# UM-Applied-Algorithms-Lab/AWRY

Measured on NVIDIA B200. Metric: count queries/s, higher is better.
Workload: dtype u32

## Files before the change

### awry_b200/csrc/batch.cu

```cuda
#include "host.hpp"

using namespace awry;
using namespace awry::host;

namespace awry {
namespace host {


static bool trace_on() {
  static const bool on = getenv("AWRY_B200_TRACE") != nullptr;
  return on;
}
static void trace_mark(const char* what, long long i = -1) {
  if (!trace_on()) return;
  static const auto t_origin = std::chrono::steady_clock::now();
  fprintf(stderr, "[trace] %10.3f ms  %s %lld\n",
          std::chrono::duration<double, std::milli>(std::chrono::steady_clock::now() - t_origin).count(), what, i);
}
struct GpuTrace {
  struct Ev {
    cudaEvent_t e;
    const char* what;
    long long i;
  };
// ... 160 lines not shown
  host_parallel_blocks(size_t(nb), [&](size_t b) {
    if (!ok.load(std::memory_order_relaxed)) return;
    const uint64_t lo = b * BLK, hi = std::min(nq, lo + BLK);
    uint64_t bad = 0;
    for (uint64_t i = lo; i <= hi; i++) bad |= off[i] ^ (first + i * l);
    if (bad) ok.store(false, std::memory_order_relaxed);
  });
  return ok.load();
}

void enqueue_search(const awry_index* ix, Replica& r, PackBalance& bal, Workspace* ws, const QuerySource& qs,
                    const Chunk& c, SearchOut mode, bool may_pack = true, bool probe_link = false, bool copy_flag = true,
                    void* d_out_override = nullptr) {
  const uint64_t nq = c.q1 - c.q0, nbytes = c.b1 - c.b0;
  const size_t out_elem = mode == OUT_COUNT_U64 ? 8 : mode == OUT_RANGE_U64 ? 16 : sp_cnt_bytes(r.view);
  const int ush = packed_unit_shift(ix->alphabet);
  Workspace::grow_dev(ws->d_qbytes, ws->d_qbytes_cap, size_t(nbytes) + 16);
  Workspace::grow_dev(ws->d_qoff, ws->d_qoff_cap, size_t(nq) + 1);
  Workspace::grow_dev(ws->d_qwords, ws->d_qwords_cap, size_t(packed_words(ix->alphabet, nq, nbytes)));
  Workspace::grow_dev(ws->d_out, ws->d_out_cap, size_t(nq) * out_elem);
  Workspace::grow_dev(ws->d_defer, ws->d_defer_cap, defer_words(nq));
  const uint64_t* src_o = qs.qoff + c.q0;
  uint64_t* const d_words = ws->d_qwords - 4 * (c.b0 >> ush);
  ws->link_probe_bytes = 0;
  uint64_t uni_len = 0;
  const bool uniform = offsets_are_uniform(src_o, nq, uni_len);
  auto upload_offsets = [&] {
    if (uniform) {
      CU(launch_fill_offsets(ws->d_qoff, c.b0, uni_len, nq, ws->st));
    } else {
      CU(cudaMemcpyAsync(ws->d_qoff, src_o, (nq + 1) * 8, cudaMemcpyHostToDevice, ws->st));
      g_prof.h2d += (nq + 1) * 8;
    }
  };
  auto stage_offsets = [&] {
    if (qs.pinned || uniform) return;
    Workspace::grow_host(ws->h_qoff, ws->h_qoff_cap, size_t(nq) + 1);
    parallel_memcpy(ws->h_qoff, src_o, (nq + 1) * 8);
    src_o = ws->h_qoff;
  };
  if (qs.crumbs) {
    const uint64_t cb0 = c.b0 >> 2, cb1 = (c.b1 + 3) >> 2;
    const size_t pbytes = size_t(cb1 - cb0);
    const uint8_t* src_c = qs.crumbs + cb0;
    const uint64_t* e_lo = std::lower_bound(qs.exc, qs.exc + qs.n_exc, c.b0 << 8);
    const uint64_t* e_hi = std::lower_bound(e_lo, qs.exc + qs.n_exc, c.b1 << 8);
// ... 59 lines not shown
    } else {
      if (!qs.pinned) {
        Workspace::grow_host(ws->h_qbytes, ws->h_qbytes_cap, size_t(nbytes) + 16);
        parallel_memcpy(ws->h_qbytes, src_b, nbytes);
        src_b = ws->h_qbytes;
      }
      stage_offsets();
      const bool probe = probe_link && qs.pinned && nbytes >= (8u << 20);
      if (probe) {
        if (!ws->ev_a) {
          CU(cudaEventCreate(&ws->ev_a));
          CU(cudaEventCreate(&ws->ev_b));
        }
        CU(cudaEventRecord(ws->ev_a, ws->st));
      }
      if (nbytes) CU(cudaMemcpyAsync(ws->d_qbytes, src_b, nbytes, cudaMemcpyHostToDevice, ws->st));
      if (probe) {
        CU(cudaEventRecord(ws->ev_b, ws->st));
        ws->link_probe_bytes = nbytes;
      }
      upload_offsets();
      g_prof.h2d += nbytes;
      CU(cudaMemsetAsync(ws->d_flag, 0xff, 8, ws->st));
      {
        ProfScope p(2, r.device, ws->st);
        CU(launch_pack(ix->alphabet, ws->d_qbytes - c.b0, ws->d_qoff, nq, d_words, c.b0, c.b1, ws->d_flag, ws->st));
      }
    }
  }
  gpu_mark(ws->st, "packed on device", (long long)c.q0);
  {
    ProfScope p(0, r.device, ws->st);
    SearchVariant v = current_variant();
    v.avg_len = uint32_t(std::min<uint64_t>(nbytes / std::max<uint64_t>(1, nq), 1u << 30));
    v.b_lo = c.b0;
    v.b_hi = c.b1;
    v.locate_positions = mode == OUT_SP_CNT_U32 && locate_positions_ok(r.view, v);
    ws->sp_cnt_positions = v.locate_positions;
    ws->gpu_probe_bytes = 0;
    const bool time_kernel = qs.pinned && !qs.crumbs && nbytes >= (8u << 20);
    if (time_kernel) {
      if (!ws->ev_s0) {
        CU(cudaEventCreate(&ws->ev_s0));
        CU(cudaEventCreate(&ws->ev_s1));
      }
      CU(cudaEventRecord(ws->ev_s0, ws->st));
    }
    CU(launch_search(r.view, d_words, ws->d_qoff, nq, mode, d_out_override ? d_out_override : ws->d_out, ws->d_defer, v,
                     r.sm_count, ws->st));
    if (time_kernel) {
      CU(cudaEventRecord(ws->ev_s1, ws->st));
      ws->gpu_probe_bytes = nbytes;
    }
  }
  gpu_mark(ws->st, "searched", (long long)c.q0);
  if (copy_flag) CU(cudaMemcpyAsync(ws->h_flag, ws->d_flag, 8, cudaMemcpyDeviceToHost, ws->st));
  trace_mark("  search enqueued, queries", (long long)nq);
}

[[noreturn]] void fail_bad_query(unsigned long long code, uint64_t q_base) {
  const unsigned long long q = q_base + (code >> 1);
  if ((code & 1) == BAD_OFFSETS)
    fail(AWRY_ERR_INVALID_ARG, "query offsets are not monotone at query %llu (its bytes lie outside the batch)", q);
  fail(AWRY_ERR_INVALID_QUERY,
       "query %llu is empty or contains a sentinel ('$'/'#'): the reference panics on it "
       "(fm_index.rs:406, bwt.rs:127)", q);
}

void check_flag(Workspace* ws, const Chunk& c) {
  if (*ws->h_flag != ~0ull) fail_bad_query(*ws->h_flag, c.q0);
}

// ... 969 lines not shown
  });
}

int awry_count_device(const awry_index* ix, int replica, const uint8_t* d_qbytes, const uint64_t* d_qoff, uint64_t nq,
                      uint64_t* d_counts, void* cuda_stream) {
  return guarded([&] {
    need(ix);
    if (replica < 0 || size_t(replica) >= ix->reps.size()) fail(AWRY_ERR_INVALID_ARG, "replica out of range");
    if (nq == 0) return;
    if (!d_qbytes || !d_qoff || !d_counts) fail(AWRY_ERR_INVALID_ARG, "null argument");
    Replica& r = *ix->reps[size_t(replica)];
    DeviceGuard dg(r.device);
    cudaStream_t st = static_cast<cudaStream_t>(cuda_stream);
    uint64_t ends[2] = {0, 0};
    CU(cudaMemcpyAsync(&ends[0], d_qoff, 8, cudaMemcpyDeviceToHost, st));
    CU(cudaMemcpyAsync(&ends[1], d_qoff + nq, 8, cudaMemcpyDeviceToHost, st));
    CU(cudaStreamSynchronize(st));
    if (ends[1] < ends[0]) fail(AWRY_ERR_INVALID_ARG, "query offsets are not monotone");
    const int sh = packed_unit_shift(ix->alphabet);
    uint64_t words = 4 * (nq + ((ends[1] >> sh) - (ends[0] >> sh)) + 2) + 32;
    uint64_t* d_qwords = nullptr;
    CU(cudaMallocAsync(reinterpret_cast<void**>(&d_qwords), words * 8 + defer_words(nq) * 4, st));
    uint32_t* d_defer = reinterpret_cast<uint32_t*>(d_qwords + words);
    {
      ProfScope p(2, r.device, st);
      CU(launch_pack(ix->alphabet, d_qbytes, d_qoff, nq, d_qwords - 4 * (ends[0] >> sh), ends[0], ends[1], r.d_async_flag, st));
    }
    {
      ProfScope p(0, r.device, st);
      SearchVariant v = current_variant();
      v.avg_len = uint32_t(std::min<uint64_t>((ends[1] - ends[0]) / nq, 1u << 30));
      v.b_lo = ends[0];
      v.b_hi = ends[1];
      CU(launch_search(r.view, d_qwords - 4 * (ends[0] >> sh), d_qoff, nq, OUT_COUNT_U64, d_counts, d_defer, v, r.sm_count, st));
    }
    CU(cudaFreeAsync(d_qwords, st));
  });
}

int awry_locate_device(const awry_index* ix, int replica, const uint8_t* d_qbytes, const uint64_t* d_qoff, uint64_t nq,
                       uint32_t flags, uint64_t* d_hit_off, awry_hit** d_hits, uint64_t* n_hits, void* cuda_stream) {
  return guarded([&] {
    need(ix);
    if (replica < 0 || size_t(replica) >= ix->reps.size()) fail(AWRY_ERR_INVALID_ARG, "replica out of range");
    if (!d_hit_off || !d_hits || !n_hits) fail(AWRY_ERR_INVALID_ARG, "null argument");
    *d_hits = nullptr;
    *n_hits = 0;
    if (nq == 0) return;
    if (!d_qbytes || !d_qoff) fail(AWRY_ERR_INVALID_ARG, "null argument");
    Replica& r = *ix->reps[size_t(replica)];
    DeviceGuard dg(r.device);
    cudaStream_t st = static_cast<cudaStream_t>(cuda_stream);
    uint64_t ends[2] = {0, 0};
    CU(cudaMemcpyAsync(&ends[0], d_qoff, 8, cudaMemcpyDeviceToHost, st));
    CU(cudaMemcpyAsync(&ends[1], d_qoff + nq, 8, cudaMemcpyDeviceToHost, st));
    CU(cudaStreamSynchronize(st));
    if (ends[1] < ends[0]) fail(AWRY_ERR_INVALID_ARG, "query offsets are not monotone");
    const int sh = packed_unit_shift(ix->alphabet);
    Workspace* ws = r.acquire();
    try {
      uint64_t words = 4 * (nq + ((ends[1] >> sh) - (ends[0] >> sh)) + 2) + 32;
      Workspace::grow_dev(ws->d_qwords, ws->d_qwords_cap, size_t(words));
      Workspace::grow_dev(ws->d_out, ws->d_out_cap, size_t(nq) * sp_cnt_bytes(r.view));
      Workspace::grow_dev(ws->d_defer, ws->d_defer_cap, defer_words(nq));
      {
        ProfScope p(2, r.device, st);
        CU(launch_pack(ix->alphabet, d_qbytes, d_qoff, nq, ws->d_qwords - 4 * (ends[0] >> sh), ends[0], ends[1], r.d_async_flag, st));
      }
      {
        ProfScope p(0, r.device, st);
        SearchVariant v = current_variant();
        v.avg_len = uint32_t(std::min<uint64_t>((ends[1] - ends[0]) / nq, 1u << 30));
        v.b_lo = ends[0];
        v.b_hi = ends[1];
        v.locate_positions = locate_positions_ok(r.view, v);
        ws->sp_cnt_positions = v.locate_positions;
        CU(launch_search(r.view, ws->d_qwords - 4 * (ends[0] >> sh), d_qoff, nq, OUT_SP_CNT_U32, ws->d_out, ws->d_defer, v, r.sm_count, st));
      }
      uint64_t n = 0;
      uint64_t* h = locate_chunk_device(ix, r, ws, nq, flags, d_hit_off, &n, st);
      CU(cudaStreamSynchronize(st));
      *d_hits = reinterpret_cast<awry_hit*>(h);
      *n_hits = n;
    } catch (...) {
      cudaStreamSynchronize(st);
      r.release(ws);
      throw;
    }
    r.release(ws);
  });
}

int awry_count_batch_hamming(const awry_index* ix, const uint8_t* qbytes, const uint64_t* qoff, uint64_t nq,
                             uint32_t max_mismatches, uint64_t* counts) {
  return guarded([&] {
    need(ix);
    if (max_mismatches > AWRY_HAMMING_MAX) fail(AWRY_ERR_INVALID_ARG, "max_mismatches must be 0 .. %d", AWRY_HAMMING_MAX);
    if (nq == 0) return;
    if (!qbytes || !qoff || !counts) fail(AWRY_ERR_INVALID_ARG, "null argument");
    hamming_check_index(ix);
// ... 150 lines not shown
```

### awry_b200/csrc/kernels.cu

```cuda
#include <atomic>
#include <cstdio>
#include <cub/device/device_scan.cuh>
#include <cub/device/device_segmented_sort.cuh>
#include <thrust/iterator/counting_iterator.h>
#include <thrust/iterator/transform_iterator.h>

#include "kernels_common.cuh"

namespace awry {

std::atomic<uint64_t> g_launches{0};
uint64_t kernel_launch_count() { return g_launches.load(); }
void kernel_launch_count_reset() { g_launches.store(0); }


__constant__ uint8_t c_ascii_to_dsym[2][256];
__constant__ uint8_t c_amino_code_to_idx[32];

static uint8_t host_ascii_to_ref_index(int alphabet, uint8_t ch) {
  if (ch >= 'a' && ch <= 'z') ch = uint8_t(ch - 'a' + 'A');
  if (ch == '$' || ch == '#') return 0;
  if (alphabet == 0) {
    switch (ch) {
      case 'A': return 1;
// ... 480 lines not shown
  return cleanup(e);
}


template <int ALPHA>
__device__ __forceinline__ uint64_t pack_word_bytes(const uint8_t* __restrict__ src, uint32_t len, uint32_t first,
                                                    const uint8_t* lut, bool& bad) {
  constexpr int BITS = ALPHA == 0 ? 4 : 8;
  constexpr int SPW = 64 / BITS;
  constexpr uint32_t SENT = ALPHA == 0 ? DNA_SENTINEL : AMINO_SENTINEL;
  uint64_t word = 0;
#pragma unroll 4
  for (int t = 0; t < SPW; t++) {
    uint32_t si = first + t;
    if (si < len) {
      uint32_t d = lut[src[len - 1 - si]];
      bad |= d == SENT;
      word |= uint64_t(d) << (BITS * t);
    }
  }
  return word;
}

template <int ALPHA, int PL = 8>
__global__ void __launch_bounds__(256)
    pack_kernel(const uint8_t* __restrict__ qbytes, const uint64_t* __restrict__ qoff, uint64_t nq,
                uint64_t* __restrict__ qwords, uint64_t b_lo, uint64_t b_hi, unsigned long long* first_bad) {
  constexpr int SPW = ALPHA == 0 ? 16 : 8;
  constexpr int LOG_SPW = ALPHA == 0 ? 4 : 3;
  constexpr int UNIT_SHIFT = ALPHA == 0 ? 6 : 5;
  __shared__ uint8_t lut[256];
  lut[threadIdx.x] = c_ascii_to_dsym[ALPHA][threadIdx.x];
  __syncthreads();
  constexpr int LOG_PL = PL == 8 ? 3 : PL == 4 ? 2 : 1;
  const uint32_t sub = threadIdx.x & (PL - 1);
  const uint64_t ngroups = (gridDim.x * uint64_t(blockDim.x)) >> LOG_PL;
  for (uint64_t q = (blockIdx.x * uint64_t(blockDim.x) + threadIdx.x) >> LOG_PL; q < nq; q += ngroups) {
    const uint64_t o0 = qoff[q], o1 = qoff[q + 1];
    if (o0 < b_lo || o1 > b_hi || o1 < o0 || o1 - o0 >= (1ull << 32)) {
      if (sub == 0) atomicMin(first_bad, bad_query_code(q, BAD_OFFSETS));
      continue;
    }
    if (o1 == o0) {
      if (sub == 0) atomicMin(first_bad, bad_query_code(q, BAD_QUERY));
      continue;
    }
// ... 1 lines not shown
    const uint32_t nwords = (len + SPW - 1) >> LOG_SPW;
    uint64_t* const dst = qwords + 4 * (q + (o0 >> UNIT_SHIFT));
    const uint8_t* const src = qbytes + o0;
    bool bad = false;
#pragma unroll 4
    for (uint32_t wi = sub; wi < nwords; wi += PL) {
      const uint32_t first = wi << LOG_SPW;
      uint64_t word;
      bool done = false;
      if (ALPHA == 0 && len >= 16) {
        const uint32_t have = len - first;
        const uint32_t drop = have >= 16 ? 0 : 16 - have;
        const uint8_t* p = src + (have >= 16 ? have - 16 : 0);
        const uint32_t sh = uint32_t(reinterpret_cast<uintptr_t>(p) & 3);
        const uint32_t* a = reinterpret_cast<const uint32_t*>(p - sh);
        uint32_t u[5];
#pragma unroll
        for (int j = 0; j < 4; j++) u[j] = __ldg(a + j);
        u[4] = sh ? __ldg(a + 4) : 0u;
        uint32_t nibs[4];
        bool clean = true;
#pragma unroll
        for (int j = 0; j < 4; j++) {
          uint32_t w4 = __funnelshift_r(u[j], u[j + 1], 8 * sh);
          uint32_t rev = __byte_perm(w4, 0, 0x0123);
          uint32_t up = rev & 0xDFDFDFDFu;
          uint32_t x4 = (up >> 1) & 0x03030303u;
          uint32_t c4 = x4 ^ ((x4 >> 1) & 0x01010101u);
          uint32_t sel = c4 | (c4 >> 4);
          uint32_t nib = (sel & 0xffu) | ((sel >> 8) & 0xff00u);
          clean &= up == __byte_perm(0x54474341u, 0, nib);
          nibs[j] = nib;
        }
        if (clean) {
          word = (uint64_t(nibs[1] | (nibs[0] << 16)) << 32) | uint64_t(nibs[3] | (nibs[2] << 16));
          word >>= 4 * drop;
          done = true;
        }
      }
      if (!done) word = pack_word_bytes<ALPHA>(src, len, first, lut, bad);
      dst[wi] = word;
    }
    if (bad) atomicMin(first_bad, bad_query_code(q, BAD_QUERY));
  }
}

cudaError_t launch_pack(int alphabet, const uint8_t* d_qbytes, const uint64_t* d_qoff, uint64_t nq,
                        uint64_t* d_qwords, uint64_t b_lo, uint64_t b_hi, unsigned long long* d_first_bad,
                        cudaStream_t s) {
  if (nq == 0) return cudaSuccess;
  const uint64_t avg_len = b_hi != ~0ull && b_hi > b_lo ? (b_hi - b_lo) / nq : 150;
  const int pl = alphabet != 0 ? 8 : avg_len >= 48 ? 4 : 2;
  uint64_t threads = nq * uint64_t(pl);
  unsigned grid = unsigned(std::min<uint64_t>((threads + 255) / 256, 148 * 64));
  if (alphabet == 0 && pl == 4)
// ... 553 lines not shown
          for (uint32_t sec = s_first + sub; sec <= s_last; sec += 4) {
            AWRY_CHK(uint64_t(sec) * 32 + 31 < ix.n_rtext);
            const u32x8 t = ldg256(ix.rtext + size_t(sec) * 32);
            bad |= in_ring ? text_sector_mismatch<true>(t, ring, sec, rb0, done, len)
                           : text_sector_mismatch<false>(t, qwords + ubase, sec, rb0, done, len);
          }
          ok = !__any_sync(gmask, bad != 0u);
        }
        if (sub == 0) {
          if (MODE == OUT_COUNT_U64)
            reinterpret_cast<uint64_t*>(out)[cur] = ok ? 1ull : 0ull;
          else
            reinterpret_cast<uint2*>(out)[cur] = ok ? make_uint2(p - left, CNT_AT_TEXT_POS) : make_uint2(1u, 0u);
        }
        cur = NONE;
        left = 0;
      }
    }
  }
}

constexpr int WAVE_MAX_STEPS = 6;

template <int MODE, int TPB, int MINB>
__global__ void __launch_bounds__(TPB, MINB)
    search_dna_wave_kernel(IndexView ix, const uint64_t* __restrict__ qwords, const uint64_t* __restrict__ qoff,
                           uint64_t nq, void* __restrict__ out, uint32_t* __restrict__ defer, uint32_t ticket_sz,
                           ByteRange br) {
  constexpr uint32_t FULL = 0xffffffffu;
  enum : uint32_t { W_NONE = 0, W_RUN = 1, W_EMPTY = 2 };
  __shared__ uint64_t s_q[TPB / 4][16];
  const uint32_t lane = threadIdx.x & 31, sub = lane & 3, gbase = lane - sub, gmask = 0xfu << gbase, grp = lane >> 2;
  uint64_t* const ring = s_q[threadIdx.x >> 2];
  const uint32_t nq32 = uint32_t(nq);
  uint32_t* const ticket = defer + nq + 1;
  uint32_t* const rest = defer + nq + 2;
  uint32_t pn = 0, pe = 0;
  uint32_t ahead = 0;
  if (lane == 0) ahead = atomicAdd(ticket, ticket_sz);
  for (;;) {
    if (pn == pe) {
      uint32_t t = ahead;
      if (lane == 0 && t < nq32) ahead = atomicAdd(ticket, ticket_sz);
      t = __shfl_sync(FULL, t, 0);
      if (t >= nq32) break;
      pn = t;
      pe = t + (nq32 - t < ticket_sz ? nq32 - t : ticket_sz);
    }
    const uint32_t q = pn + grp;
    uint32_t st = q < pe ? W_RUN : W_NONE;
    pn = pe - pn > 8u ? pn + 8u : pe;

    uint64_t ov = 0;
    if (st == W_RUN) ov = __ldg(qoff + q + (sub & 1));
    const uint64_t o0 = __shfl_sync(FULL, ov, gbase), o1 = __shfl_sync(FULL, ov, gbase + 1);
    const uint32_t len = st == W_RUN ? checked_len(o0, o1, br) : 0u;
    if (st == W_RUN && len == 0) st = W_EMPTY;
    const uint32_t nwords = (len + 15) >> 4;
    if (st == W_RUN && nwords > 16) {
      if (sub == 0) rest[2 + atomicAdd(rest, 1u)] = q;
      st = W_NONE;
    }
    uint32_t amb = 0;
    __syncwarp();
    if (st == W_RUN && 4 * sub < nwords) {
      const uint32_t ubase = 4 * (q + uint32_t(o0 >> 6));
      AWRY_CHK_QWORDS(ubase + 4 * sub, br, nq, 6);
      const u32x8 t = ldg256(qwords + ubase + 4 * sub);
#pragma unroll
      for (int j = 0; j < 4; j++) {
        ring[4 * sub + j] = uint64_t(t.v[2 * j]) | (uint64_t(t.v[2 * j + 1]) << 32);
        if (4 * sub + j < nwords) amb |= (t.v[2 * j] | t.v[2 * j + 1]) & 0xCCCCCCCCu;
      }
    }
    const uint32_t amb_groups = __ballot_sync(FULL, amb != 0);
    __syncwarp();
    if (st == W_RUN && (amb_groups & gmask) != 0) {
      if (sub == 0) defer[1 + atomicAdd(defer, 1u)] = q;
      st = W_NONE;
    }
    uint32_t sp = 1, ep = 0, left = 0;
    if (st == W_RUN) {
      const uint32_t k = ix.kmer_len;
      const uint64_t w = ring[0];
      if (k != 0 && len >= k) {
        const uint64_t idx = kmer_index(w, k);
        AWRY_CHK(idx < ix.n_table);
        const uint2 r = __ldg(ix.table + idx);
        sp = r.x;
        ep = r.y;
        left = len - k;
      } else {
        const uint32_t c = uint32_t(w) & 15u;
        sp = ix.c_lo[c];
        ep = ix.c_hi[c];
        left = len - 1;
      }
    }
#pragma unroll 1
    for (int it = 0; it <= WAVE_MAX_STEPS; it++) {
      const bool active = st == W_RUN && left != 0 && sp <= ep && !(sp == ep && left >= VERIFY_MIN_LEFT);
      if (!__any_sync(FULL, active)) break;
      if (it == WAVE_MAX_STEPS) {
        if (active) {
          if (sub == 0) rest[2 + atomicAdd(rest, 1u)] = q;
          st = W_NONE;
        }
        break;
      }
      const uint32_t pos = len - left;
      const uint8_t* const rb8 = reinterpret_cast<const uint8_t*>(ring);
      const uint32_t qb = rb8[(pos >> 1) & 127];
      const bool two = left >= 2;
      const uint32_t pa = sp - 1, pb = ep;
      uint32_t ra = 0, rb = 0, base = 0;
      if (active) {
        if (two) {
          const uint32_t q2 = ((qb | (uint32_t(rb8[((pos >> 1) + 1) & 127]) << 8)) >> (4 * (pos & 1))) & 0xffu;
          const uint32_t pair = ((q2 & 3u) << 2) | (q2 >> 4);
          const uint32_t ba = __umulhi(pa, 0xAAAAAAABu) >> 6, bb = __umulhi(pb, 0xAAAAAAABu) >> 6;
          AWRY_CHK(uint64_t(ba) * PAIR_BLOCK_UINT4 + 7 < ix.n_pair_u4 && uint64_t(bb) * PAIR_BLOCK_UINT4 + 7 < ix.n_pair_u4);
          const u32x8 x = ldg256(ix.pair_blocks + size_t(ba) * PAIR_BLOCK_UINT4 + 2 * sub);
          u32x8 y = x;
          if (bb != ba) y = ldg256(ix.pair_blocks + size_t(bb) * PAIR_BLOCK_UINT4 + 2 * sub);
          PairSlice s = pair_slice(x, sub, pair);
          ra = __popc(s.match & low_mask(int(pa - ba * PAIR_ROWS_PER_BLOCK) + 1 - int(32 * sub))) + s.count;
          if (bb != ba) s = pair_slice(y, sub, pair);
// ... 348 lines not shown
  int per_sm = 0;
  cudaError_t e = cudaOccupancyMaxActiveBlocksPerMultiprocessor(&per_sm, kern, TPB, 0);
  if (e != cudaSuccess) return e;
  if (per_sm < 1) per_sm = 1;
  if (force_per_sm > 0 && force_per_sm < per_sm) per_sm = force_per_sm;
  uint64_t max_blocks = uint64_t(sm_count) * uint64_t(per_sm);
  uint64_t need_blocks = (nq * 4 + TPB - 1) / TPB;
  unsigned grid = unsigned(std::max<uint64_t>(1, std::min(max_blocks, need_blocks)));
  static const uint32_t ticket_env = [] {
    if (const char* e = getenv("AWRY_B200_TICKET")) return uint32_t(std::min(1024l, std::max(1l, strtol(e, nullptr, 10))));
    return 0u;
  }();
  uint32_t per_group = avg_len == 0 ? 2u : std::min(8u, std::max(1u, 200u / avg_len));
  per_group = ticket_cap(per_group, nq, uint64_t(grid) * (TPB / 4), avg_len);
  const uint32_t ticket_sz = ticket_env ? ticket_env : 8u * per_group;
  e = launch_with_table_window(kern, grid, TPB, s, ix, ix, d_qwords, d_qoff, nq, d_out, d_defer, ticket_sz, br);
  COUNT_LAUNCH();
  if (e != cudaSuccess) return e;
  search_scalar_kernel<0, MODE, true><<<unsigned(sm_count) * 2, 256, 0, s>>>(ix, d_qwords, d_qoff, nq, d_out, d_defer, br);
  COUNT_LAUNCH();
  return cudaGetLastError();
}

template <int MODE>
static cudaError_t launch_search_wave(const IndexView& ix, const uint64_t* d_qwords, const uint64_t* d_qoff, uint64_t nq,
                                      void* d_out, uint32_t* d_defer, int sm_count, cudaStream_t s, uint32_t avg_len,
                                      ByteRange br) {
  constexpr int TPB = 256, MINB = 6;
  cudaError_t e = cudaMemsetAsync(d_defer + nq + 2, 0, 8, s);
  if (e != cudaSuccess) return e;
  auto kern = search_dna_wave_kernel<MODE, TPB, MINB>;
  auto kern_rest = search_dna_pair_kernel<MODE, TPB, 4, true, true>;
  int per_sm = 0, per_sm_rest = 0;
  if ((e = cudaOccupancyMaxActiveBlocksPerMultiprocessor(&per_sm, kern, TPB, 0)) != cudaSuccess) return e;
  if ((e = cudaOccupancyMaxActiveBlocksPerMultiprocessor(&per_sm_rest, kern_rest, TPB, 0)) != cudaSuccess) return e;
  const uint64_t need_blocks = (nq * 4 + TPB - 1) / TPB;
  const unsigned grid = unsigned(std::max<uint64_t>(1, std::min<uint64_t>(uint64_t(sm_count) * std::max(1, per_sm), need_blocks)));
  const unsigned grid_rest = unsigned(std::max<uint64_t>(1, std::min<uint64_t>(uint64_t(sm_count) * std::max(1, per_sm_rest), need_blocks)));
  static const uint32_t ticket_env = [] {
    if (const char* e = getenv("AWRY_B200_TICKET")) return uint32_t(std::min(1024l, std::max(8l, strtol(e, nullptr, 10)))) & ~7u;
    return 0u;
  }();
  uint32_t ticket_sz = nq >= uint64_t(grid) * (TPB / 32) * 128 ? 32u : 8u;
  if (ticket_env) ticket_sz = ticket_env;
  e = launch_with_table_window(kern, grid, TPB, s, ix, ix, d_qwords, d_qoff, nq, d_out, d_defer, ticket_sz, br);
  COUNT_LAUNCH();
  if (e != cudaSuccess) return e;
  uint32_t per_group = avg_len == 0 ? 2u : std::min(8u, std::max(1u, 200u / avg_len));
  e = launch_with_table_window(kern_rest, grid_rest, TPB, s, ix, ix, d_qwords, d_qoff, nq, d_out, d_defer, 8u * per_group, br);
  COUNT_LAUNCH();
  if (e != cudaSuccess) return e;
  search_scalar_kernel<0, MODE, true><<<unsigned(sm_count) * 2, 256, 0, s>>>(ix, d_qwords, d_qoff, nq, d_out, d_defer, br);
  COUNT_LAUNCH();
  return cudaGetLastError();
}

template <int MODE, int MINB, int NS, bool VFY = false>
static cudaError_t launch_search_pairx_b(const IndexView& ix, const uint64_t* d_qwords, const uint64_t* d_qoff,
                                         uint64_t nq, void* d_out, uint32_t* d_defer, int sm_count, cudaStream_t s,
                                         uint32_t avg_len, ByteRange br) {
  constexpr int TPB = 256;
  auto kern = search_dna_pairx_kernel<MODE, TPB, MINB, NS, VFY>;
  int per_sm = 0;
  cudaError_t e = cudaOccupancyMaxActiveBlocksPerMultiprocessor(&per_sm, kern, TPB, 0);
  if (e != cudaSuccess) return e;
  if (per_sm < 1) per_sm = 1;
  const uint64_t max_blocks = uint64_t(sm_count) * uint64_t(per_sm);
  const uint64_t need_blocks = (nq * 4 + uint64_t(TPB) * NS - 1) / (uint64_t(TPB) * NS);
  const unsigned grid = unsigned(std::max<uint64_t>(1, std::min(max_blocks, need_blocks)));
  static const uint32_t ticket_env = [] {
    if (const char* e = getenv("AWRY_B200_TICKET")) return uint32_t(std::min(1024l, std::max(1l, strtol(e, nullptr, 10))));
    return 0u;
  }();
  uint32_t per_slot = avg_len == 0 ? 2u : std::min(8u, std::max(1u, 200u / avg_len));
  per_slot = ticket_cap(per_slot, nq, uint64_t(grid) * (TPB / 4) * NS, avg_len);
  const uint32_t ticket_sz = ticket_env ? ticket_env : 8u * NS * per_slot;
  e = launch_with_table_window(kern, grid, TPB, s, ix, ix, d_qwords, d_qoff, nq, d_out, d_defer, ticket_sz, br);
  COUNT_LAUNCH();
  if (e != cudaSuccess) return e;
  search_scalar_kernel<0, MODE, true><<<unsigned(sm_count) * 2, 256, 0, s>>>(ix, d_qwords, d_qoff, nq, d_out, d_defer, br);
  COUNT_LAUNCH();
  return cudaGetLastError();
}

template <int MODE>
static cudaError_t launch_search_pair(const IndexView& ix, const uint64_t* d_qwords, const uint64_t* d_qoff,
                                      uint64_t nq, void* d_out, uint32_t* d_defer, const SearchVariant& v,
                                      int sm_count, cudaStream_t s) {
  if (nq >= (1ull << 32) - (1u << 24)) return cudaErrorInvalidValue;
  cudaError_t e = cudaMemsetAsync(d_defer, 0, 4, s);
  if (e != cudaSuccess) return e;
  e = cudaMemsetAsync(d_defer + nq + 1, 0, 4, s);
  if (e != cudaSuccess) return e;
  const ByteRange br{v.b_lo, v.b_hi};
  static const int slots_default = [] {
    if (const char* e = getenv("AWRY_B200_SLOTS")) return std::max(0, std::min(4, atoi(e)));
    return 0;
  }();
  const int slots = v.slots >= 0 ? v.slots : slots_default;
  const bool in_text = v.finish_in_text && ix.rtext != nullptr && ix.full_sa != nullptr &&
                       (MODE == OUT_COUNT_U64 || (MODE == OUT_SP_CNT_U32 && v.locate_positions));
  if (in_text && v.slots < 0 && slots_default == 0 && v.blocks_per_sm == 0) {
    if (MODE == OUT_COUNT_U64) return launch_search_wave<OUT_COUNT_U64>(ix, d_qwords, d_qoff, nq, d_out, d_defer, sm_count, s, v.avg_len, br);
    if (MODE == OUT_SP_CNT_U32) return launch_search_wave<OUT_SP_CNT_U32>(ix, d_qwords, d_qoff, nq, d_out, d_defer, sm_count, s, v.avg_len, br);
  }
  if (MODE == OUT_SP_CNT_U32 && in_text)
    return launch_search_pair_b<OUT_SP_CNT_U32, 5, true>(ix, d_qwords, d_qoff, nq, d_out, d_defer, 0, sm_count, s, v.avg_len, br);
  if (MODE == OUT_COUNT_U64 && in_text) {
    if (slots == 1) return launch_search_pairx_b<OUT_COUNT_U64, 8, 1, true>(ix, d_qwords, d_qoff, nq, d_out, d_defer, sm_count, s, v.avg_len, br);
    if (slots == 2) return launch_search_pairx_b<OUT_COUNT_U64, 5, 2, true>(ix, d_qwords, d_qoff, nq, d_out, d_defer, sm_count, s, v.avg_len, br);
    if (slots == 3) return launch_search_pairx_b<OUT_COUNT_U64, 6, 1, true>(ix, d_qwords, d_qoff, nq, d_out, d_defer, sm_count, s, v.avg_len, br);
    if (slots == 4) return launch_search_pairx_b<OUT_COUNT_U64, 4, 2, true>(ix, d_qwords, d_qoff, nq, d_out, d_defer, sm_count, s, v.avg_len, br);
    switch (v.blocks_per_sm) {
      case 4: return launch_search_pair_b<OUT_COUNT_U64, 4, true>(ix, d_qwords, d_qoff, nq, d_out, d_defer, 0, sm_count, s, v.avg_len, br);
      case 6: return launch_search_pair_b<OUT_COUNT_U64, 6, true>(ix, d_qwords, d_qoff, nq, d_out, d_defer, 0, sm_count, s, v.avg_len, br);
      case 8: return launch_search_pair_b<OUT_COUNT_U64, 8, true>(ix, d_qwords, d_qoff, nq, d_out, d_defer, 0, sm_count, s, v.avg_len, br);
      default: return launch_search_pair_b<OUT_COUNT_U64, 5, true>(ix, d_qwords, d_qoff, nq, d_out, d_defer, 0, sm_count, s, v.avg_len, br);
    }
  }
  if (slots == 1 || slots == 3) return launch_search_pairx_b<MODE, 8, 1>(ix, d_qwords, d_qoff, nq, d_out, d_defer, sm_count, s, v.avg_len, br);
  if (slots == 2 || slots == 4) return launch_search_pairx_b<MODE, 5, 2>(ix, d_qwords, d_qoff, nq, d_out, d_defer, sm_count, s, v.avg_len, br);
  switch (v.blocks_per_sm) {
    case 4: return launch_search_pair_b<MODE, 4>(ix, d_qwords, d_qoff, nq, d_out, d_defer, 0, sm_count, s, v.avg_len, ByteRange{v.b_lo, v.b_hi});
    case 8: return launch_search_pair_b<MODE, 8>(ix, d_qwords, d_qoff, nq, d_out, d_defer, 0, sm_count, s, v.avg_len, ByteRange{v.b_lo, v.b_hi});
    case 0:
// ... 381 lines not shown
                                      int sm_count, cudaStream_t s) {
  if (ix.alphabet == 0 && v.lanes != -1) {
    if (ix.pair_blocks != nullptr && (v.lanes == 0 || v.lanes == 8))
      return launch_search_pair<MODE>(ix, d_qwords, d_qoff, nq, d_out, d_defer, v, sm_count, s);
    switch (v.lanes) {
      case 1: return launch_search_dna<1, MODE>(ix, d_qwords, d_qoff, nq, d_out, v, sm_count, s);
      case 4: return launch_search_dna<4, MODE>(ix, d_qwords, d_qoff, nq, d_out, v, sm_count, s);
      default: return launch_search_dna<2, MODE>(ix, d_qwords, d_qoff, nq, d_out, v, sm_count, s);
    }
  }
  if (ix.alphabet == 1 && v.lanes != -1)
    return launch_search_amino<MODE>(ix, d_qwords, d_qoff, nq, d_out, d_defer, v, sm_count, s);
  int per_sm = 8;
  uint64_t need_blocks = (nq + 255) / 256;
  unsigned grid = unsigned(std::max<uint64_t>(1, std::min<uint64_t>(uint64_t(sm_count) * per_sm, need_blocks)));
  if (ix.alphabet == 0)
    search_scalar_kernel<0, MODE, false><<<grid, 256, 0, s>>>(ix, d_qwords, d_qoff, nq, d_out, nullptr, ByteRange{v.b_lo, v.b_hi});
  else
    search_scalar_kernel<1, MODE, false><<<grid, 256, 0, s>>>(ix, d_qwords, d_qoff, nq, d_out, nullptr, ByteRange{v.b_lo, v.b_hi});
  COUNT_LAUNCH();
  return cudaGetLastError();
}

cudaError_t launch_search(const IndexView& ix, const uint64_t* d_qwords, const uint64_t* d_qoff,
                          uint64_t nq, SearchOut mode, void* d_out, uint32_t* d_defer,
                          const SearchVariant& v, int sm_count, cudaStream_t s) {
  if (nq == 0) return cudaSuccess;
  if (ix.wide) return launch_search_wide(*ix.wide, d_qwords, d_qoff, nq, mode, d_out, d_defer, v, sm_count, s);
  switch (mode) {
    case OUT_COUNT_U64: return launch_search_mode<OUT_COUNT_U64>(ix, d_qwords, d_qoff, nq, d_out, d_defer, v, sm_count, s);
    case OUT_RANGE_U64: return launch_search_mode<OUT_RANGE_U64>(ix, d_qwords, d_qoff, nq, d_out, d_defer, v, sm_count, s);
    default: return launch_search_mode<OUT_SP_CNT_U32>(ix, d_qwords, d_qoff, nq, d_out, d_defer, v, sm_count, s);
  }
}

}
```

### awry_b200/csrc/kernels.hpp

```cpp
#pragma once
#include <algorithm>
#include <cstdint>
#include <cuda_runtime.h>

#include "layout.cuh"

namespace awry {

inline uint64_t packed_words(int alphabet, uint64_t nq, uint64_t total_bytes) {
  return 4 * (nq + (total_bytes >> (alphabet == 0 ? 6 : 5)) + 2) + 32;
}
inline int packed_unit_shift(int alphabet) { return alphabet == 0 ? 6 : 5; }

enum SearchOut { OUT_COUNT_U64 = 0, OUT_RANGE_U64 = 1, OUT_SP_CNT_U32 = 2 };
constexpr uint32_t CNT_AT_TEXT_POS = 0xffffffffu;

struct SearchVariant {
  int lanes = 0;
  int tpb = 0;
  int blocks_per_sm = 0;
  int slots = -1;
  bool finish_in_text = true;
  bool locate_positions = false;
  uint32_t avg_len = 0;
// ... 38 lines not shown
cudaError_t launch_fill_offsets(uint64_t* d_qoff, uint64_t first, uint64_t len, uint64_t n, cudaStream_t s);
cudaError_t build_full_sa(const IndexView& ix, uint32_t* d_full, int sm_count, cudaStream_t s);
inline size_t rtext_bytes(int alphabet, uint64_t bwt_len) {
  return ((alphabet == 0 ? (size_t(bwt_len) + 1) / 2 : size_t(bwt_len)) + 127) / 128 * 128 + 128;
}
cudaError_t build_rtext(const IndexView& ix, uint8_t* d_rtext, cudaStream_t s);

enum BadKind : unsigned { BAD_QUERY = 0, BAD_OFFSETS = 1 };
__host__ __device__ inline unsigned long long bad_query_code(uint64_t q, unsigned kind) { return (q << 1) | kind; }
uint64_t walk_block_count(uint64_t bwt_len);
cudaError_t build_lean_sa(const IndexView& ix, uint4* d_walk, uint32_t* d_rank, uint32_t* d_pos, int sm_count,
                          cudaStream_t s);

cudaError_t launch_pack(int alphabet, const uint8_t* d_qbytes, const uint64_t* d_qoff, uint64_t nq,
                        uint64_t* d_qwords, uint64_t b_lo, uint64_t b_hi, unsigned long long* d_first_bad,
                        cudaStream_t s);
cudaError_t launch_pack2(const uint32_t* d_crumbs, uint64_t base, const uint64_t* d_qoff, uint64_t nq, uint64_t* d_qwords,
                         const uint64_t* d_exc, uint64_t n_exc, uint64_t exc_base, uint64_t b_lo, uint64_t b_hi,
                         unsigned long long* d_first_bad, cudaStream_t s);
inline size_t defer_words(uint64_t nq) { return 2 * size_t(nq) + 8; }
cudaError_t launch_search(const IndexView& ix, const uint64_t* d_qwords, const uint64_t* d_qoff,
                          uint64_t nq, SearchOut mode, void* d_out, uint32_t* d_defer,
                          const SearchVariant& v, int sm_count, cudaStream_t s);

cudaError_t scan_hit_offsets(const IndexView& ix, const void* d_sp_cnt, uint64_t nq, uint64_t* d_hit_off, void* d_temp,
                             size_t& temp_bytes, cudaStream_t s);
inline size_t sp_cnt_bytes(const IndexView& ix) { return ix.wide ? 16 : 8; }
cudaError_t launch_walk(const IndexView& ix, const void* d_sp_cnt, const uint64_t* d_hit_off,
                        uint64_t nq, uint64_t n_hits, uint64_t* d_hits_pairs, uint64_t* d_locs,
                        int sm_count, cudaStream_t s);
cudaError_t launch_gather_direct(const IndexView& ix, const uint2* d_sp_cnt, const uint64_t* d_local_off, uint64_t nq,
                                 unsigned long long* d_running, unsigned long long* d_chunk_base, void* out_hits,
                                 uint64_t capacity, uint64_t* d_off_out, int sm_count, cudaEvent_t wait_before_advance,
                                 cudaEvent_t record_after_advance, cudaStream_t s);
cudaError_t sort_hit_segments(uint64_t* d_locs_in, uint64_t* d_locs_out, uint64_t n_hits,
                              uint64_t nq, const uint64_t* d_hit_off, void* d_temp,
                              size_t& temp_bytes, cudaStream_t s);
cudaError_t launch_map_locations(const IndexView& ix, const uint64_t* d_locs, uint64_t n_hits,
                                 uint64_t* d_hits_pairs, cudaStream_t s);

cudaError_t launch_hamming_pieces(const uint64_t* d_qoff, uint64_t nq, uint32_t k, uint64_t b_lo, uint64_t b_hi,
                                  uint64_t* d_poff, unsigned long long* d_first_bad, cudaStream_t s);
cudaError_t launch_hamming_query_bounds(const uint64_t* d_hoff, uint32_t k, uint64_t nq, uint64_t* d_qcand, cudaStream_t s);
cudaError_t launch_hamming_map(const uint64_t* d_hoff, uint64_t npieces, uint64_t c0, uint64_t n, uint32_t* d_map,
                               void* d_temp, size_t& temp_bytes, cudaStream_t s);
struct HammingSlice {
// ... 48 lines not shown
```

Before: 5.053 billion.

## Fuse ASCII-to-nibble query packing into the DNA wave search kernel

When the wave search kernel applies, the separate pack kernel is skipped. The search kernel now reads raw ASCII query bytes directly, converts them to nibbles into its shared ring, and writes packed words only for queries that fall back to the deferred or rest kernels. This removes one kernel launch and a full write and read of the packed query buffer. The cost is extra work in the search kernel, added register and shared-memory pressure (a 256-byte LUT), and more complex validation for bad queries.

Result: faster. 6.140 billion, median of 6 (+21.5%).

```diff
diff --git a/awry_b200/csrc/batch.cu b/awry_b200/csrc/batch.cu
--- a/awry_b200/csrc/batch.cu
+++ b/awry_b200/csrc/batch.cu
@@ -206,6 +206,12 @@
   Workspace::grow_dev(ws->d_defer, ws->d_defer_cap, defer_words(nq));
   const uint64_t* src_o = qs.qoff + c.q0;
   uint64_t* const d_words = ws->d_qwords - 4 * (c.b0 >> ush);
+  SearchVariant v = current_variant();
+  v.avg_len = uint32_t(std::min<uint64_t>(nbytes / std::max<uint64_t>(1, nq), 1u << 30));
+  v.b_lo = c.b0;
+  v.b_hi = c.b1;
+  v.locate_positions = mode == OUT_SP_CNT_U32 && locate_positions_ok(r.view, v);
+  bool in_wave = false;
   ws->link_probe_bytes = 0;
   uint64_t uni_len = 0;
   const bool uniform = offsets_are_uniform(src_o, nq, uni_len);
@@ -311,7 +317,8 @@
       upload_offsets();
       g_prof.h2d += nbytes;
       CU(cudaMemsetAsync(ws->d_flag, 0xff, 8, ws->st));
-      {
+      in_wave = search_packs_ascii(r.view, mode, v);
+      if (!in_wave) {
         ProfScope p(2, r.device, ws->st);
         CU(launch_pack(ix->alphabet, ws->d_qbytes - c.b0, ws->d_qoff, nq, d_words, c.b0, c.b1, ws->d_flag, ws->st));
       }
@@ -320,11 +327,6 @@
   gpu_mark(ws->st, "packed on device", (long long)c.q0);
   {
     ProfScope p(0, r.device, ws->st);
-    SearchVariant v = current_variant();
-    v.avg_len = uint32_t(std::min<uint64_t>(nbytes / std::max<uint64_t>(1, nq), 1u << 30));
-    v.b_lo = c.b0;
-    v.b_hi = c.b1;
-    v.locate_positions = mode == OUT_SP_CNT_U32 && locate_positions_ok(r.view, v);
     ws->sp_cnt_positions = v.locate_positions;
     ws->gpu_probe_bytes = 0;
     const bool time_kernel = qs.pinned && !qs.crumbs && nbytes >= (8u << 20);
@@ -335,8 +337,12 @@
       }
       CU(cudaEventRecord(ws->ev_s0, ws->st));
     }
-    CU(launch_search(r.view, d_words, ws->d_qoff, nq, mode, d_out_override ? d_out_override : ws->d_out, ws->d_defer, v,
-                     r.sm_count, ws->st));
+    void* const d_out = d_out_override ? d_out_override : ws->d_out;
+    if (in_wave)
+      CU(launch_search_ascii(r.view, ws->d_qbytes - c.b0, ws->d_qoff, nq, d_words, ws->d_flag, mode, d_out, ws->d_defer, v,
+                             r.sm_count, ws->st));
+    else
+      CU(launch_search(r.view, d_words, ws->d_qoff, nq, mode, d_out, ws->d_defer, v, r.sm_count, ws->st));
     if (time_kernel) {
       CU(cudaEventRecord(ws->ev_s1, ws->st));
       ws->gpu_probe_bytes = nbytes;
@@ -1352,17 +1358,23 @@
     uint64_t* d_qwords = nullptr;
     CU(cudaMallocAsync(reinterpret_cast<void**>(&d_qwords), words * 8 + defer_words(nq) * 4, st));
     uint32_t* d_defer = reinterpret_cast<uint32_t*>(d_qwords + words);
-    {
+    uint64_t* const d_words = d_qwords - 4 * (ends[0] >> sh);
+    SearchVariant v = current_variant();
+    v.avg_len = uint32_t(std::min<uint64_t>((ends[1] - ends[0]) / nq, 1u << 30));
+    v.b_lo = ends[0];
+    v.b_hi = ends[1];
+    const bool in_wave = search_packs_ascii(r.view, OUT_COUNT_U64, v);
+    if (!in_wave) {
       ProfScope p(2, r.device, st);
-      CU(launch_pack(ix->alphabet, d_qbytes, d_qoff, nq, d_qwords - 4 * (ends[0] >> sh), ends[0], ends[1], r.d_async_flag, st));
+      CU(launch_pack(ix->alphabet, d_qbytes, d_qoff, nq, d_words, ends[0], ends[1], r.d_async_flag, st));
     }
     {
       ProfScope p(0, r.device, st);
-      SearchVariant v = current_variant();
-      v.avg_len = uint32_t(std::min<uint64_t>((ends[1] - ends[0]) / nq, 1u << 30));
-      v.b_lo = ends[0];
-      v.b_hi = ends[1];
-      CU(launch_search(r.view, d_qwords - 4 * (ends[0] >> sh), d_qoff, nq, OUT_COUNT_U64, d_counts, d_defer, v, r.sm_count, st));
+      if (in_wave)
+        CU(launch_search_ascii(r.view, d_qbytes, d_qoff, nq, d_words, r.d_async_flag, OUT_COUNT_U64, d_counts, d_defer, v,
+                               r.sm_count, st));
+      else
+        CU(launch_search(r.view, d_words, d_qoff, nq, OUT_COUNT_U64, d_counts, d_defer, v, r.sm_count, st));
     }
     CU(cudaFreeAsync(d_qwords, st));
   });
@@ -1393,19 +1405,25 @@
       Workspace::grow_dev(ws->d_qwords, ws->d_qwords_cap, size_t(words));
       Workspace::grow_dev(ws->d_out, ws->d_out_cap, size_t(nq) * sp_cnt_bytes(r.view));
       Workspace::grow_dev(ws->d_defer, ws->d_defer_cap, defer_words(nq));
-      {
+      uint64_t* const d_words = ws->d_qwords - 4 * (ends[0] >> sh);
+      SearchVariant v = current_variant();
+      v.avg_len = uint32_t(std::min<uint64_t>((ends[1] - ends[0]) / nq, 1u << 30));
+      v.b_lo = ends[0];
+      v.b_hi = ends[1];
+      v.locate_positions = locate_positions_ok(r.view, v);
+      ws->sp_cnt_positions = v.locate_positions;
+      const bool in_wave = search_packs_ascii(r.view, OUT_SP_CNT_U32, v);
+      if (!in_wave) {
         ProfScope p(2, r.device, st);
-        CU(launch_pack(ix->alphabet, d_qbytes, d_qoff, nq, ws->d_qwords - 4 * (ends[0] >> sh), ends[0], ends[1], r.d_async_flag, st));
+        CU(launch_pack(ix->alphabet, d_qbytes, d_qoff, nq, d_words, ends[0], ends[1], r.d_async_flag, st));
       }
       {
         ProfScope p(0, r.device, st);
-        SearchVariant v = current_variant();
-        v.avg_len = uint32_t(std::min<uint64_t>((ends[1] - ends[0]) / nq, 1u << 30));
-        v.b_lo = ends[0];
-        v.b_hi = ends[1];
-        v.locate_positions = locate_positions_ok(r.view, v);
-        ws->sp_cnt_positions = v.locate_positions;
-        CU(launch_search(r.view, ws->d_qwords - 4 * (ends[0] >> sh), d_qoff, nq, OUT_SP_CNT_U32, ws->d_out, ws->d_defer, v, r.sm_count, st));
+        if (in_wave)
+          CU(launch_search_ascii(r.view, d_qbytes, d_qoff, nq, d_words, r.d_async_flag, OUT_SP_CNT_U32, ws->d_out,
+                                 ws->d_defer, v, r.sm_count, st));
+        else
+          CU(launch_search(r.view, d_words, d_qoff, nq, OUT_SP_CNT_U32, ws->d_out, ws->d_defer, v, r.sm_count, st));
       }
       uint64_t n = 0;
       uint64_t* h = locate_chunk_device(ix, r, ws, nq, flags, d_hit_off, &n, st);
diff --git a/awry_b200/csrc/kernels.cu b/awry_b200/csrc/kernels.cu
--- a/awry_b200/csrc/kernels.cu
+++ b/awry_b200/csrc/kernels.cu
@@ -526,6 +526,17 @@
   return word;
 }
 
+__device__ __forceinline__ uint32_t ascii4_to_nibbles(uint32_t w4, uint32_t& diff) {
+  const uint32_t rev = __byte_perm(w4, 0, 0x0123);
+  const uint32_t up = rev & 0xDFDFDFDFu;
+  const uint32_t x4 = (up >> 1) & 0x03030303u;
+  const uint32_t c4 = x4 ^ ((x4 >> 1) & 0x01010101u);
+  const uint32_t sel = c4 | (c4 >> 4);
+  const uint32_t nib = (sel & 0xffu) | ((sel >> 8) & 0xff00u);
+  diff = up ^ __byte_perm(0x54474341u, 0, nib);
+  return nib;
+}
+
 template <int ALPHA, int PL = 8>
 __global__ void __launch_bounds__(256)
     pack_kernel(const uint8_t* __restrict__ qbytes, const uint64_t* __restrict__ qoff, uint64_t nq,
@@ -573,15 +584,9 @@
         bool clean = true;
 #pragma unroll
         for (int j = 0; j < 4; j++) {
-          uint32_t w4 = __funnelshift_r(u[j], u[j + 1], 8 * sh);
-          uint32_t rev = __byte_perm(w4, 0, 0x0123);
-          uint32_t up = rev & 0xDFDFDFDFu;
-          uint32_t x4 = (up >> 1) & 0x03030303u;
-          uint32_t c4 = x4 ^ ((x4 >> 1) & 0x01010101u);
-          uint32_t sel = c4 | (c4 >> 4);
-          uint32_t nib = (sel & 0xffu) | ((sel >> 8) & 0xff00u);
-          clean &= up == __byte_perm(0x54474341u, 0, nib);
-          nibs[j] = nib;
+          uint32_t diff;
+          nibs[j] = ascii4_to_nibbles(__funnelshift_r(u[j], u[j + 1], 8 * sh), diff);
+          clean &= diff == 0;
         }
         if (clean) {
           word = (uint64_t(nibs[1] | (nibs[0] << 16)) << 32) | uint64_t(nibs[3] | (nibs[2] << 16));
@@ -1181,14 +1186,78 @@
 
 constexpr int WAVE_MAX_STEPS = 6;
 
-template <int MODE, int TPB, int MINB>
+__device__ __forceinline__ uint32_t stage_ascii_ring(uintptr_t b, uintptr_t e, bool run, uint32_t sub, uint32_t gbase,
+                                                     uint64_t* ring) {
+  constexpr uint32_t FULL = 0xffffffffu;
+  const uint32_t nsec = run ? uint32_t(((e - 1) >> 5) - (b >> 5)) + 1 : 0u;
+  const uintptr_t end32 = (e + 31) & ~uintptr_t(31);
+  const uint32_t pad = uint32_t(end32 - e), ph = pad >> 3, pl4 = 4 * (pad & 7);
+  uint32_t* const r32 = reinterpret_cast<uint32_t*>(ring);
+  uint32_t dirty = 0, carry = 0;
+  const int rounds = int(__reduce_max_sync(FULL, (nsec + 3) >> 2));
+#pragma unroll 1
+  for (int i = rounds - 1; i >= 0; i--) {
+    const uint32_t k = sub + 4u * uint32_t(i);
+    uint32_t h[5] = {0u, 0u, 0u, 0u, 0u};
+    if (k < nsec) {
+      const u32x8 t = ldg256(reinterpret_cast<const void*>(end32 - 32 * uintptr_t(k + 1)));
+      uint32_t nib[8];
+#pragma unroll
+      for (int j = 0; j < 8; j++) {
+        uint32_t diff;
+        nib[j] = ascii4_to_nibbles(t.v[j], diff);
+        dirty |= diff;
+      }
+      h[0] = nib[7] | (nib[6] << 16);
+      h[1] = nib[5] | (nib[4] << 16);
+      h[2] = nib[3] | (nib[2] << 16);
+      h[3] = nib[1] | (nib[0] << 16);
+    }
+    const uint32_t x = __shfl_sync(FULL, h[0], gbase + ((sub + 1) & 3));
+    h[4] = sub == 3 ? carry : x;
+    carry = x;
+    if (k < nsec) {
+#pragma unroll
+      for (int j = 0; j < 4; j++) {
+        const int m = int(4 * k) - int(ph) + j;
+        if (m >= 0 && m < 32) r32[m] = __funnelshift_r(h[j], h[j + 1], pl4);
+      }
+    }
+  }
+  return dirty;
+}
+
+__device__ __forceinline__ uint32_t read_is_dirty(const uint8_t* src, uint32_t len, uint32_t sub) {
+  uint32_t dirty = 0;
+  for (uint32_t i = sub; i < len; i += 4) {
+    uint32_t diff;
+    ascii4_to_nibbles(0x41414100u | src[i], diff);
+    dirty |= diff;
+  }
+  return dirty;
+}
+
+__device__ __forceinline__ void pack_query_lut(const uint8_t* src, uint32_t len, uint32_t nwords, uint64_t* dst,
+                                               uint32_t sub, const uint8_t* lut, uint64_t q, unsigned long long* first_bad) {
+  bool bad = false;
+  for (uint32_t wi = sub; wi < nwords; wi += 4) dst[wi] = pack_word_bytes<0>(src, len, wi << 4, lut, bad);
+  if (bad) atomicMin(first_bad, bad_query_code(q, BAD_QUERY));
+}
+
+template <int MODE, int TPB, int MINB, bool ASCII = false>
 __global__ void __launch_bounds__(TPB, MINB)
     search_dna_wave_kernel(IndexView ix, const uint64_t* __restrict__ qwords, const uint64_t* __restrict__ qoff,
                            uint64_t nq, void* __restrict__ out, uint32_t* __restrict__ defer, uint32_t ticket_sz,
-                           ByteRange br) {
+                           ByteRange br, const uint8_t* __restrict__ qbytes, uint64_t* qw_out,
+                           unsigned long long* first_bad) {
   constexpr uint32_t FULL = 0xffffffffu;
   enum : uint32_t { W_NONE = 0, W_RUN = 1, W_EMPTY = 2 };
   __shared__ uint64_t s_q[TPB / 4][16];
+  __shared__ uint8_t s_lut[ASCII ? 256 : 1];
+  if (ASCII) {
+    s_lut[threadIdx.x] = c_ascii_to_dsym[0][threadIdx.x];
+    __syncthreads();
+  }
   const uint32_t lane = threadIdx.x & 31, sub = lane & 3, gbase = lane - sub, gmask = 0xfu << gbase, grp = lane >> 2;
   uint64_t* const ring = s_q[threadIdx.x >> 2];
   const uint32_t nq32 = uint32_t(nq);
@@ -1214,16 +1283,25 @@
     if (st == W_RUN) ov = __ldg(qoff + q + (sub & 1));
     const uint64_t o0 = __shfl_sync(FULL, ov, gbase), o1 = __shfl_sync(FULL, ov, gbase + 1);
     const uint32_t len = st == W_RUN ? checked_len(o0, o1, br) : 0u;
-    if (st == W_RUN && len == 0) st = W_EMPTY;
+    if (st == W_RUN && len == 0) {
+      st = W_EMPTY;
+      if (ASCII && sub == 0)
+        atomicMin(first_bad, bad_query_code(q, o1 == o0 && o0 >= br.lo && o1 <= br.hi ? BAD_QUERY : BAD_OFFSETS));
+    }
     const uint32_t nwords = (len + 15) >> 4;
+    const uint32_t ubase = 4 * (q + uint32_t(o0 >> 6));
     if (st == W_RUN && nwords > 16) {
+      if (ASCII) pack_query_lut(qbytes + o0, len, nwords, qw_out + ubase, sub, s_lut, q, first_bad);
       if (sub == 0) rest[2 + atomicAdd(rest, 1u)] = q;
       st = W_NONE;
     }
     uint32_t amb = 0;
     __syncwarp();
-    if (st == W_RUN && 4 * sub < nwords) {
-      const uint32_t ubase = 4 * (q + uint32_t(o0 >> 6));
+    if (ASCII) {
+      amb = stage_ascii_ring(uintptr_t(qbytes + o0), uintptr_t(qbytes + o1), st == W_RUN, sub, gbase, ring);
+      const uint32_t dirty_groups = __ballot_sync(FULL, amb != 0);
+      if (dirty_groups) amb = st == W_RUN && (dirty_groups & gmask) ? read_is_dirty(qbytes + o0, len, sub) : 0u;
+    } else if (st == W_RUN && 4 * sub < nwords) {
       AWRY_CHK_QWORDS(ubase + 4 * sub, br, nq, 6);
       const u32x8 t = ldg256(qwords + ubase + 4 * sub);
 #pragma unroll
@@ -1235,6 +1313,7 @@
     const uint32_t amb_groups = __ballot_sync(FULL, amb != 0);
     __syncwarp();
     if (st == W_RUN && (amb_groups & gmask) != 0) {
+      if (ASCII) pack_query_lut(qbytes + o0, len, nwords, qw_out + ubase, sub, s_lut, q, first_bad);
       if (sub == 0) defer[1 + atomicAdd(defer, 1u)] = q;
       st = W_NONE;
     }
@@ -1262,6 +1341,16 @@
       if (!__any_sync(FULL, active)) break;
       if (it == WAVE_MAX_STEPS) {
         if (active) {
+          if (ASCII) {
+#pragma unroll
+            for (uint32_t j = 4 * sub; j < 4 * sub + 4; j++) {
+              if (j < nwords) {
+                AWRY_CHK_QWORDS(ubase + j, br, nq, 6);
+                const uint32_t tail = len - 16 * j;
+                qw_out[ubase + j] = tail >= 16 ? ring[j] : ring[j] & ((1ull << (4 * tail)) - 1);
+              }
+            }
+          }
           if (sub == 0) rest[2 + atomicAdd(rest, 1u)] = q;
           st = W_NONE;
         }
@@ -1656,14 +1745,20 @@
   return cudaGetLastError();
 }
 
-template <int MODE>
+struct AsciiQueries {
+  const uint8_t* qbytes = nullptr;
+  uint64_t* qwords = nullptr;
+  unsigned long long* first_bad = nullptr;
+};
+
+template <int MODE, bool ASCII = false>
 static cudaError_t launch_search_wave(const IndexView& ix, const uint64_t* d_qwords, const uint64_t* d_qoff, uint64_t nq,
                                       void* d_out, uint32_t* d_defer, int sm_count, cudaStream_t s, uint32_t avg_len,
-                                      ByteRange br) {
+                                      ByteRange br, const AsciiQueries& a = AsciiQueries()) {
   constexpr int TPB = 256, MINB = 6;
   cudaError_t e = cudaMemsetAsync(d_defer + nq + 2, 0, 8, s);
   if (e != cudaSuccess) return e;
-  auto kern = search_dna_wave_kernel<MODE, TPB, MINB>;
+  auto kern = search_dna_wave_kernel<MODE, TPB, MINB, ASCII>;
   auto kern_rest = search_dna_pair_kernel<MODE, TPB, 4, true, true>;
   int per_sm = 0, per_sm_rest = 0;
   if ((e = cudaOccupancyMaxActiveBlocksPerMultiprocessor(&per_sm, kern, TPB, 0)) != cudaSuccess) return e;
@@ -1677,7 +1772,8 @@
   }();
   uint32_t ticket_sz = nq >= uint64_t(grid) * (TPB / 32) * 128 ? 32u : 8u;
   if (ticket_env) ticket_sz = ticket_env;
-  e = launch_with_table_window(kern, grid, TPB, s, ix, ix, d_qwords, d_qoff, nq, d_out, d_defer, ticket_sz, br);
+  e = launch_with_table_window(kern, grid, TPB, s, ix, ix, d_qwords, d_qoff, nq, d_out, d_defer, ticket_sz, br, a.qbytes,
+                               a.qwords, a.first_bad);
   COUNT_LAUNCH();
   if (e != cudaSuccess) return e;
   uint32_t per_group = avg_len == 0 ? 2u : std::min(8u, std::max(1u, 200u / avg_len));
@@ -1717,24 +1813,41 @@
   return cudaGetLastError();
 }
 
+static int slots_default() {
+  static const int d = [] {
+    if (const char* e = getenv("AWRY_B200_SLOTS")) return std::max(0, std::min(4, atoi(e)));
+    return 0;
+  }();
+  return d;
+}
+
+static bool finishes_in_text(const IndexView& ix, SearchOut mode, const SearchVariant& v) {
+  return v.finish_in_text && ix.rtext != nullptr && ix.full_sa != nullptr &&
+         (mode == OUT_COUNT_U64 || (mode == OUT_SP_CNT_U32 && v.locate_positions));
+}
+
+static bool runs_wave_kernel(const IndexView& ix, SearchOut mode, const SearchVariant& v) {
+  return !ix.wide && ix.alphabet == 0 && ix.pair_blocks != nullptr && (v.lanes == 0 || v.lanes == 8) &&
+         finishes_in_text(ix, mode, v) && v.slots < 0 && slots_default() == 0 && v.blocks_per_sm == 0;
+}
+
+static cudaError_t reset_defer(uint64_t nq, uint32_t* d_defer, cudaStream_t s) {
+  if (nq >= (1ull << 32) - (1u << 24)) return cudaErrorInvalidValue;
+  cudaError_t e = cudaMemsetAsync(d_defer, 0, 4, s);
+  if (e != cudaSuccess) return e;
+  return cudaMemsetAsync(d_defer + nq + 1, 0, 4, s);
+}
+
 template <int MODE>
 static cudaError_t launch_search_pair(const IndexView& ix, const uint64_t* d_qwords, const uint64_t* d_qoff,
                                       uint64_t nq, void* d_out, uint32_t* d_defer, const SearchVariant& v,
                                       int sm_count, cudaStream_t s) {
-  if (nq >= (1ull << 32) - (1u << 24)) return cudaErrorInvalidValue;
-  cudaError_t e = cudaMemsetAsync(d_defer, 0, 4, s);
-  if (e != cudaSuccess) return e;
-  e = cudaMemsetAsync(d_defer + nq + 1, 0, 4, s);
+  cudaError_t e = reset_defer(nq, d_defer, s);
   if (e != cudaSuccess) return e;
   const ByteRange br{v.b_lo, v.b_hi};
-  static const int slots_default = [] {
-    if (const char* e = getenv("AWRY_B200_SLOTS")) return std::max(0, std::min(4, atoi(e)));
-    return 0;
-  }();
-  const int slots = v.slots >= 0 ? v.slots : slots_default;
-  const bool in_text = v.finish_in_text && ix.rtext != nullptr && ix.full_sa != nullptr &&
-                       (MODE == OUT_COUNT_U64 || (MODE == OUT_SP_CNT_U32 && v.locate_positions));
-  if (in_text && v.slots < 0 && slots_default == 0 && v.blocks_per_sm == 0) {
+  const int slots = v.slots >= 0 ? v.slots : slots_default();
+  const bool in_text = finishes_in_text(ix, SearchOut(MODE), v);
+  if (runs_wave_kernel(ix, SearchOut(MODE), v)) {
     if (MODE == OUT_COUNT_U64) return launch_search_wave<OUT_COUNT_U64>(ix, d_qwords, d_qoff, nq, d_out, d_defer, sm_count, s, v.avg_len, br);
     if (MODE == OUT_SP_CNT_U32) return launch_search_wave<OUT_SP_CNT_U32>(ix, d_qwords, d_qoff, nq, d_out, d_defer, sm_count, s, v.avg_len, br);
   }
@@ -2162,6 +2275,28 @@
   return cudaGetLastError();
 }
 
+bool search_packs_ascii(const IndexView& ix, SearchOut mode, const SearchVariant& v) {
+  const char* e = getenv("AWRY_B200_ASCII_WAVE");
+  return !(e && e[0] == '0') && runs_wave_kernel(ix, mode, v);
+}
+
+cudaError_t launch_search_ascii(const IndexView& ix, const uint8_t* d_qbytes, const uint64_t* d_qoff, uint64_t nq,
+                                uint64_t* d_qwords, unsigned long long* d_first_bad, SearchOut mode, void* d_out,
+                                uint32_t* d_defer, const SearchVariant& v, int sm_count, cudaStream_t s) {
+  if (nq == 0) return cudaSuccess;
+  if (!runs_wave_kernel(ix, mode, v)) return cudaErrorInvalidValue;
+  cudaError_t e = reset_defer(nq, d_defer, s);
+  if (e != cudaSuccess) return e;
+  const ByteRange br{v.b_lo, v.b_hi};
+  AsciiQueries a;
+  a.qbytes = d_qbytes;
+  a.qwords = d_qwords;
+  a.first_bad = d_first_bad;
+  if (mode == OUT_COUNT_U64)
+    return launch_search_wave<OUT_COUNT_U64, true>(ix, d_qwords, d_qoff, nq, d_out, d_defer, sm_count, s, v.avg_len, br, a);
+  return launch_search_wave<OUT_SP_CNT_U32, true>(ix, d_qwords, d_qoff, nq, d_out, d_defer, sm_count, s, v.avg_len, br, a);
+}
+
 cudaError_t launch_search(const IndexView& ix, const uint64_t* d_qwords, const uint64_t* d_qoff,
                           uint64_t nq, SearchOut mode, void* d_out, uint32_t* d_defer,
                           const SearchVariant& v, int sm_count, cudaStream_t s) {
diff --git a/awry_b200/csrc/kernels.hpp b/awry_b200/csrc/kernels.hpp
--- a/awry_b200/csrc/kernels.hpp
+++ b/awry_b200/csrc/kernels.hpp
@@ -84,6 +84,10 @@
 cudaError_t launch_search(const IndexView& ix, const uint64_t* d_qwords, const uint64_t* d_qoff,
                           uint64_t nq, SearchOut mode, void* d_out, uint32_t* d_defer,
                           const SearchVariant& v, int sm_count, cudaStream_t s);
+bool search_packs_ascii(const IndexView& ix, SearchOut mode, const SearchVariant& v);
+cudaError_t launch_search_ascii(const IndexView& ix, const uint8_t* d_qbytes, const uint64_t* d_qoff, uint64_t nq,
+                                uint64_t* d_qwords, unsigned long long* d_first_bad, SearchOut mode, void* d_out,
+                                uint32_t* d_defer, const SearchVariant& v, int sm_count, cudaStream_t s);
 
 cudaError_t scan_hit_offsets(const IndexView& ix, const void* d_sp_cnt, uint64_t nq, uint64_t* d_hit_off, void* d_temp,
                              size_t& temp_bytes, cudaStream_t s);
```
